# Arbol-Project/dcdf

Hardware: AMD Instinct MI355X
Metric: raster cells/s encoded (Snapshot+Log build) (higher is better)
Workload: dtype int32; 1 GPU; configs[2]: 4096x4096x365 i32 raster, seed 0xDCDF0003, tiled into 3072 [<=32,256,256] chunks; 3072 of them on this GPU; workload_key=config2/i32/n3072/w1, chunks_total=3072, chunks_on_rank0=3072, cells_total=6123683840, k=2, device=gfx950:sramecc+:xnack- AMD Radeon Graphics, 256 CUs, failed_tiles_rank0=0, encoded_bytes_rank0=4115239087, snapshots_rank0=3072, bytes_verified_vs_oracle=0, parallelism=chunks sharded over 1 GPU(s), no data-path collective

## Files before the change

### dcdf_amd/csrc/k2r_encode.h

```cpp
#pragma once
#include "k2r_exec.h"


#ifndef K2R_DIAG_SKIP
#define K2R_DIAG_SKIP 0
#endif

namespace k2r {

template <int LOG2S>
struct EncCfg {
    static_assert(LOG2S >= 3 && LOG2S <= 8, "kernel body written for sidelen 8..256 (the library dispatches 16..256)");
    static constexpr int H = LOG2S;
    static constexpr int S = 1 << LOG2S;
    static constexpr int NBLK = 1 << (2 * (LOG2S - 3));
    static constexpr int NT = NBLK;
    static constexpr int NW = NT < 64 ? 1 : NT / 64;
    static constexpr int NTOP = ((1 << (2 * (H - 2))) - 1) / 3;
    static constexpr int NTOPX = NTOP - (1 << (2 * (H - 3)));
    static constexpr int TBW = (NTOPX + 31) / 32 + 1;
    static constexpr int MAXV = ((1 << (2 * (H + 1))) - 1) / 3;
    static constexpr int MAXT = ((1 << (2 * H)) - 1) / 3;
    static constexpr int WV = (MAXV + 31) / 32;
    static constexpr int WT = (MAXT + 31) / 32;
    static constexpr int top_off(int h) { return ((1 << (2 * (H - 2))) - (1 << (2 * (H - h + 1)))) / 3; }
    static constexpr int kWaveHeader = 1;
    static constexpr int kWavePrefix = 2;
};

struct EncRegs {
    uint32_t d2[4];
    uint32_t flags;
    uint32_t u2;
    uint32_t sc[MAX_SCAN_FIELDS];
    uint64_t pf_lo;
    uint32_t pf_l2;
    uint32_t pa[5];
#ifdef K2R_REGCOPY
    uint32_t cw[32];
#endif
};

K2R_HD uint32_t unpackI(int h, uint64_t lo, uint64_t top) {
    switch (h) {
        case 1: return (uint32_t)(lo & 0xffffu);
        case 2: return (uint32_t)((lo >> 16) & 0x3fffu);
        case 3: return (uint32_t)((lo >> 30) & 0xfffu);
        case 4: return (uint32_t)(top & 0x3ffu);
        case 5: return (uint32_t)((top >> 10) & 0xffu);
        case 6: return (uint32_t)((top >> 18) & 0x3fu);
// ... 511 lines not shown
};

template <class C>
struct EncShared : EncPool<C> {
    using EncPool<C>::POOL_L1;
    using EncPool<C>::POOL_BMV1;
    using EncPool<C>::POOL_PREFV;
    using EncPool<C>::POOLW;
    int32_t tmin[C::NTOP], tmax[C::NTOP], smin[C::NTOP], smax[C::NTOP], diff[C::NTOP];
    uint32_t eq[C::NTOP];
    uint32_t pool[EncPool<C>::POOLW];
    uint32_t bmT[C::WT + 1], bmE[C::WT + 1];
    uint32_t bmV0[C::WV + 1];
    uint32_t bmM[2][C::WT + 1];
    uint32_t prefM[C::WT + 2];
    uint32_t wsum[C::NW][MAX_SCAN_FIELDS];
    uint32_t tot[MAX_SCAN_FIELDS];
    K2R_HD uint32_t* L2() { return pool; }
    K2R_HD uint16_t* L1() { return (uint16_t*)(pool + POOL_L1); }
    K2R_HD uint32_t* bmV1() { return pool + POOL_BMV1; }
    K2R_HD uint32_t* prefV() { return pool + POOL_PREFV; }
    static constexpr int PREFTOP = 48;
    uint32_t prefTopV[PREFTOP + 1];
    uint32_t pfx[3][C::NBLK];
    uint32_t lq[C::NBLK][2];
    uint32_t li[C::NBLK];
    uint32_t tbS[C::TBW], tbL[C::TBW];
    uint32_t tbP[C::TBW + 1];
    uint32_t ttR[C::H + 2];
    uint32_t nlistV, nlistM;
    uint32_t stI, stQ;
    uint32_t tkI, tkQ;
    InstPlan<C> pl;
    int32_t err;
    uint32_t work;
    uint32_t fault[6];
    uint64_t prof[NPROF], prof_last;
#ifdef K2R_PROFILE
    uint64_t pw[16][NPROF][2];
#endif
};

template <class EX>
K2R_HD bool guard_ok(EX& ex, bool ok, uint32_t code, uint32_t inst, uint32_t tid, uint32_t value, uint32_t limit) {
    ex.gfail |= ok ? 0u : (1u << (code & 31u));
    (void)inst; (void)tid; (void)value; (void)limit;
    return ok;
}
template <bool UNIFORM_SPAN = true, class EX>
// ... 532 lines not shown
            o.su = 0;
#pragma unroll
            for (int q = 0; q < 4; q++) {
                x[q] = (uint32_t)((d[4 * q] ^ d[4 * q + 1]) | (d[4 * q] ^ d[4 * q + 2]) | (d[4 * q] ^ d[4 * q + 3]));
                const uint32_t u1 = nz((uint32_t)(mn1[q] ^ mx1[q]));
                o.pq[q] = u1 & nz(x[q]);
                o.tb1 = (o.tb1 << 1) | o.pq[q];
                o.e4 = (o.e4 << 1) | (u1 ^ o.pq[q]);
                o.su += u1;
                const uint32_t sxq = (q & 1) ? (sx[q >> 1] >> 16) : (sx[q >> 1] & 0xffffu);
                const uint32_t snq = (q & 1) ? (sn[q >> 1] >> 16) : (sn[q >> 1] & 0xffffu);
                o.recw[q] = pk_lo16((uint32_t)(mx1[q] - (int32_t)sxq), (uint32_t)(mn1[q] - (int32_t)snq));
                o.qw[2 * q] = pk_lo16((uint32_t)d[4 * q], (uint32_t)d[4 * q + 1]);
                o.qw[2 * q + 1] = pk_lo16((uint32_t)d[4 * q + 2], (uint32_t)d[4 * q + 3]);
            }
            const uint32_t X = x[0] | x[1] | x[2] | x[3] | (uint32_t)((d[0] ^ d[4]) | (d[0] ^ d[8]) | (d[0] ^ d[12]));
            o.ne2 = nz(X);
            o.nu2 = nz((uint32_t)(o.mn2 ^ o.mx2));
            o.p2 = o.ne2 & o.nu2;
            o.nq = popc32(o.tb1);
            o.d0 = d[0];
            o.d2w = pk_lo16((uint32_t)(o.mx2 - (int32_t)o.smx2), (uint32_t)(o.mn2 - (int32_t)o.smn2));
        };
        auto lean_put = [&](const LeanSub& o, uint32_t owner, uint32_t lI1b, uint32_t lI2b) {
            uint32_t slotQ, slotI, endQ, endI;
            ex.stash_alloc(o.nq | (o.p2 << 16), &sh.stQ, &sh.stI, slotQ, slotI, endQ, endI);
            uint32_t ord = lI1b;
            const uint32_t p0 = owner | (lI2b << 10) | (lI1b << 12) | (o.tb1 << 16) | (o.e4 << 20);
            if (endQ <= (uint32_t)SH::CAPQ_REC && endI <= (uint32_t)SH::CAPI_REC) {
#pragma unroll
                for (int q = 0; q < 4; q++) {
                    uint32_t* d = sh.pool + ((uint32_t)SH::QBASE + mul24(slotQ, 3u));
                    if (o.pq[q]) {
                        d[0] = owner | (ord << 10);
                        d[1] = o.qw[2 * q];
                        d[2] = o.qw[2 * q + 1];
                    }
                    slotQ += o.pq[q];
                    ord += o.pq[q];
                }
                if (o.p2) {
                    uint32_t* d = sh.pool + mul24(slotI, 5u);
                    d[0] = p0;
                    d[1] = o.recw[0];
                    d[2] = o.recw[1];
                    d[3] = o.recw[2];
                    d[4] = o.recw[3];
                }
            } else {
// ... 20 lines not shown
                        d[2] = o.recw[1];
                        d[3] = o.recw[2];
                        d[4] = o.recw[3];
                    } else {
                        gstore_words5(ovI + 5u * (slotI - (uint32_t)SH::CAPI_REC), p0, o.recw[0], o.recw[1], o.recw[2], o.recw[3]);
                    }
                }
            }
        };
        auto lean_block_out = [&](uint32_t B, int32_t mn3, int32_t mx3, uint32_t smn3, uint32_t smx3, int32_t dref, uint32_t Zb, uint32_t& wide,
                                  int32_t& err, bool store) {
            if (VEC == 1 && (mn3 < -VALUE_LIMIT || mx3 >= VALUE_LIMIT) && err == 0) err = ERR_RANGE;
            const int32_t smn3t = s_base + (int32_t)smn3, smx3t = s_base + (int32_t)smx3;
            wide = (mn3 - smx3t < -32768 || mx3 - smn3t > 32767) ? 1u : 0u;
            if (store) {
                sh.tmin[B] = mn3;
                sh.tmax[B] = mx3;
                if (s_build) {
                    sh.smin[B] = smn3t;
                    sh.smax[B] = smx3t;
                }
                sh.diff[B] = dref - s_base;
                sh.eq[B] = Zb == 0 ? 1u : 0u;
                sh.lq[B][0] = 0;
                sh.lq[B][1] = 0;
                sh.li[B] = 0;
            }
        };
        if (lean && !EX::kSim) {
            if constexpr (!EX::kSim) ex.par([&](int tid, EncRegs& r) {
                constexpr uint32_t NTW = NT < 64 ? NT : 64, BPP = NTW / 4;
                const uint32_t ltid = opaque((uint32_t)tid), lane = ltid & 63u, j = lane & 3u;
                int32_t err = 0;
                auto request_t = [&](int p, int32_t (&tt)[16]) {
                    const uint32_t Bp = (ltid & ~63u) + BPP * (uint32_t)p + (lane >> 2);
                    uint32_t br, bc;
                    morton_decode(4u * Bp + j, br, bc);
                    load_sub16<false, VEC>(ta, inst, 4u * br, 4u * bc, 0, tt, err);
                    if (VEC >= 2) err = (int32_t)opaque((uint32_t)err);
                };
                auto request_w = [&](int p, uint32_t (&ww)[8]) {
                    const uint32_t Bp = (ltid & ~63u) + BPP * (uint32_t)p + (lane >> 2);
#ifdef K2R_REGCOPY
#pragma unroll
                    for (int i = 0; i < 8; i++) ww[i] = r.cw[8 * p + i];
                    (void)Bp;
#else
                    load_compact_raw<C>(cmp, (int)Bp, (int)j, ww);
#endif
// ... 21 lines not shown
                    if (K2R_LEAN_PREFETCH != 1) request_w(p, w);
#pragma unroll
                    for (int i = 0; i < 16; i++) t[i] = tn[i];
                    if (K2R_LEAN_PREFETCH == 1) {
#pragma unroll
                        for (int i = 0; i < 8; i++) w[i] = wn[i];
                    }
                    if (p < 3) {
                        request_t(p + 1, tn);
                        if (K2R_LEAN_PREFETCH == 1) request_w(p + 1, wn);
                    }
                    sched_fence();
#else
                    request_t(p, t);
                    request_w(p, w);
#endif
                    LeanSub o;
                    lean_analyse(t, w, o);
                    sched_fence();
                    const uint32_t cnt = o.nq | (o.p2 << 8) | (o.su << 16) | (o.nu2 << 24);
                    const uint32_t n0 = EX::template quad_bcast<0>(cnt), n1 = EX::template quad_bcast<1>(cnt), n2 = EX::template quad_bcast<2>(cnt),
                                   n3 = EX::template quad_bcast<3>(cnt);
                    const uint32_t pre = (j > 0 ? n0 : 0u) + (j > 1 ? n1 : 0u) + (j > 2 ? n2 : 0u), tot = n0 + n1 + n2 + n3;
                    lean_put(o, B, pre & 0xffu, (pre >> 8) & 0xffu);
                    const int32_t mn3 = EX::quad_min(o.mn2), mx3 = EX::quad_max(o.mx2);
                    const uint32_t smn3 = (uint32_t)EX::quad_min((int32_t)o.smn2), smx3 = (uint32_t)EX::quad_max((int32_t)o.smx2);
                    const int32_t dref = (int32_t)EX::template quad_bcast<0>((uint32_t)o.d0);
                    const uint32_t Zb = EX::quad_or(o.ne2 | nz((uint32_t)(o.d0 ^ dref)));
                    uint32_t wide;
                    lean_block_out(B, mn3, mx3, smn3, smx3, dref, Zb, wide, err, j == 0);
                    const uint32_t fw = EX::quad_or(((o.ne2 ^ 1u) << j) | (o.su << (4u + 3u * j)) | (o.nq << (16u + 3u * j))) | (wide << 28);
                    const uint32_t uw = EX::quad_or((o.nu2 ^ 1u) << j);
                    const uint32_t own_lane = lane - BPP * (uint32_t)p, src = (4u * own_lane) & 63u;
                    const uint32_t g0 = EX::lane_pull(src, o.d2w), g1 = EX::lane_pull(src + 1u, o.d2w), g2 = EX::lane_pull(src + 2u, o.d2w),
                                   g3 = EX::lane_pull(src + 3u, o.d2w);
                    const uint32_t gf = EX::lane_pull(src, fw), gu = EX::lane_pull(src, uw), gt = EX::lane_pull(src, tot);
                    if (lane / BPP == (uint32_t)p) {
                        r.d2[0] = g0;
                        r.d2[1] = g1;
                        r.d2[2] = g2;
                        r.d2[3] = g3;
                        r.flags = gf;
                        r.u2 = gu;
                        r.sc[0] = ((gt >> 16) & 0xffu) | ((gt >> 24) << 16);
                        r.sc[3] = (gt & 0xffu) | (((gt >> 8) & 0xffu) << 16);
                    }
                }
// ... 4 lines not shown
                if (err != 0) ex.lds_min(&sh.err, err);
            });
        } else if (lean) ex.par([&](int tid, EncRegs& r) {
            uint32_t r0, c0;
            blk_origin(tid, r0, c0);
            int32_t err = 0;
            uint32_t sI1 = 0, sI2 = 0, lI1 = 0, lI2 = 0, eqbits = 0, cntbits = 0, u2 = 0, Z = 0;
            int32_t mn3 = 0, mx3 = 0, dref = 0;
            uint32_t smn3 = 0, smx3 = 0;
#pragma unroll
            for (int j = 0; j < 4; j++) {
                int32_t t[16];
                uint32_t w[8];
                load_sub16<false, VEC>(ta, inst, r0, c0, j, t, err);
#ifdef K2R_REGCOPY
                for (int i = 0; i < 8; i++) w[i] = r.cw[8 * j + i];
#else
                load_compact_raw<C>(cmp, tid, j, w);
#endif
                LeanSub o;
                lean_analyse(t, w, o);
                if (j == 0) dref = o.d0;
                Z |= o.ne2 | nz((uint32_t)(o.d0 ^ dref));
                lean_put(o, (uint32_t)tid, lI1, lI2);
                sI1 += o.su;
                sI2 += o.nu2;
                cntbits |= (o.su << (4 + 3 * j)) | (o.nq << (16 + 3 * j));
                lI1 += o.nq;
                lI2 += o.p2;
                u2 |= (o.nu2 ^ 1u) << j;
                eqbits |= (o.ne2 ^ 1u) << j;
                r.d2[j] = o.d2w;
                mn3 = j == 0 ? o.mn2 : (o.mn2 < mn3 ? o.mn2 : mn3);
                mx3 = j == 0 ? o.mx2 : (o.mx2 > mx3 ? o.mx2 : mx3);
                smn3 = j == 0 ? o.smn2 : (o.smn2 < smn3 ? o.smn2 : smn3);
                smx3 = j == 0 ? o.smx2 : (o.smx2 > smx3 ? o.smx2 : smx3);
            }
            uint32_t wide;
            lean_block_out((uint32_t)tid, mn3, mx3, smn3, smx3, dref, Z, wide, err, true);
            r.sc[0] = sI1 | (sI2 << 16);
            r.flags = eqbits | cntbits | (wide << 28);
            r.u2 = u2;
            if (tid < C::TBW) {
                sh.tbS[tid] = 0;
                sh.tbL[tid] = 0;
            }
            r.sc[3] = lI1 | (lI2 << 16);
            if (err != 0) ex.lds_min(&sh.err, err);
        });
        else ex.par([&](int tid, EncRegs& r) {
            uint32_t r0, c0;
            blk_origin(tid, r0, c0);
            int32_t err = 0;
            const bool inv3 = inval(r0, c0);
            uint32_t sI1 = 0, sI2 = 0, lI1 = 0, lI2 = 0;
            if (have_s) {
                sh.lq[tid][0] = 0;
                sh.lq[tid][1] = 0;
                sh.li[tid] = 0;
            }
            int32_t df2_0 = 0, mn3 = 0, mx3 = 0, smn3 = 0, smx3 = 0;
            uint32_t eqbits = 0, eqall = 1, cntbits = 0, wide = 0, u2 = 0;
#pragma unroll
            for (int j = 0; j < 4; j++) {
                sched_fence();
                const uint32_t rj = r0 + 4 * (j >> 1), cj = c0 + 4 * (j & 1);
                const bool inv2 = inval(rj, cj);
                int32_t t16[16];
                load_sub16<PADDED, VEC>(ta, inst, r0, c0, j, t16, err);
                int32_t mn1[4], mx1[4];
                bool inv1[4], P1S[4];
#pragma unroll
                for (int qq = 0; qq < 4; qq++) {
                    mn1[qq] = min4(t16[4 * qq], t16[4 * qq + 1], t16[4 * qq + 2], t16[4 * qq + 3]);
                    mx1[qq] = max4(t16[4 * qq], t16[4 * qq + 1], t16[4 * qq + 2], t16[4 * qq + 3]);
                    inv1[qq] = inval(rj + 2 * (qq >> 1), cj + 2 * (qq & 1));
                    P1S[qq] = !inv1[qq] && mn1[qq] != mx1[qq];
                    sI1 += P1S[qq] ? 1u : 0u;
                    cntbits += (P1S[qq] ? 1u : 0u) << (4 + 3 * j);
// ... 113 lines not shown
        ex.stamp(0);

        const bool rec_ovf = stI > (uint32_t)SH::CAPI_REC || stQ > (uint32_t)SH::CAPQ_REC;
        const uint32_t rec_corr = lean ? (uint32_t)s_base & 0xffffu : 0u;
        auto rec16 = [&](uint32_t half) -> int32_t { return (int32_t)(int16_t)(uint16_t)(half - rec_corr); };
        auto lng = [](int32_t v) -> uint32_t { return ((uint32_t)v + 128u) > 255u ? 1u : 0u; };
        auto top_node = [&](int h, int j) {
            const int c = C::top_off(h - 1) + 4 * j, a = C::top_off(h) + j;
            sh.tmin[a] = min4(sh.tmin[c], sh.tmin[c + 1], sh.tmin[c + 2], sh.tmin[c + 3]);
            sh.tmax[a] = max4(sh.tmax[c], sh.tmax[c + 1], sh.tmax[c + 2], sh.tmax[c + 3]);
            if (have_s) {
                if (s_build) {
                    sh.smin[a] = min4(sh.smin[c], sh.smin[c + 1], sh.smin[c + 2], sh.smin[c + 3]);
                    sh.smax[a] = max4(sh.smax[c], sh.smax[c + 1], sh.smax[c + 2], sh.smax[c + 3]);
                }
                const int32_t d0 = sh.diff[c];
                sh.diff[a] = d0;
                sh.eq[a] = (sh.eq[c] & sh.eq[c + 1] & sh.eq[c + 2] & sh.eq[c + 3]) && d0 == sh.diff[c + 1] && d0 == sh.diff[c + 2] &&
                                   d0 == sh.diff[c + 3]
                               ? 1u
                               : 0u;
            }
        };
        auto prepass = [&](uint32_t first, uint32_t step) {
            for (uint32_t m = first; m < stQ; m += step) {
                uint32_t q[3];
                if (m < (uint32_t)SH::CAPQ_REC) {
#pragma unroll
                    for (int i = 0; i < 3; i++) q[i] = sh.pool[SH::QBASE + 3u * m + i];
                } else {
                    gload_words<3>(ovQ + 3u * (m - (uint32_t)SH::CAPQ_REC), q);
                }
                const uint32_t own = q[0] & 1023u, ord = (q[0] >> 10) & 15u;
                const uint32_t f = lng(rec16(q[1] & 0xffffu)) | (lng(rec16(q[1] >> 16)) << 1) | (lng(rec16(q[2] & 0xffffu)) << 2) |
                                   (lng(rec16(q[2] >> 16)) << 3);
                if (f) ex.lds_or(&sh.lq[own][ord >> 3], f << (4u * (ord & 7u)));
            }
            for (uint32_t k = first; k < stI; k += step) {
                uint32_t rec[5];
                if (k < (uint32_t)SH::CAPI_REC) {
#pragma unroll
                    for (int i = 0; i < 5; i++) rec[i] = sh.pool[5u * k + i];
                } else {
                    gload_words<5>(ovI + 5u * (k - (uint32_t)SH::CAPI_REC), rec);
                }
                const uint32_t own = rec[0] & 1023u, ord2 = (rec[0] >> 10) & 3u, tb1 = (rec[0] >> 16) & 15u;
                uint32_t f = 0;
// ... 215 lines not shown
                }
            };
            const uint32_t wt = opaque((uint32_t)tid);
            node(3, wt);
            if (tid == 0) {
                sh.stI = 0;
                sh.stQ = 0;
                sh.tkI = 0;
                sh.tkQ = 0;
            }
            if (wt < (uint32_t)C::NTOPX) {
                int h;
                uint32_t j;
                top_decode(wt, h, j);
                node(h, j);
            }
            r.sc[1] = sI3 | (lI3 << 16);
            r.sc[2] = sTop;
            r.sc[4] = lTop;
            r.sc[5] = lMax.c1 | (lMin.c1 << 16);
            r.sc[6] = wide;
            uint32_t cL0 = 0, cL1 = 0, mL1 = 0, cL2 = 0, mL2 = 0;
            if (have_s) {
                const uint32_t fl = sh.li[tid];
                cL0 = popc32(sh.lq[tid][0]) + popc32(sh.lq[tid][1]);
                cL1 = popc32(fl & 0x0f0f0f0fu);
                mL1 = popc32(fl & 0xf0f0f0f0u);
#pragma unroll
                for (int j = 0; j < 4; j++) {
                    const int32_t vx = rec16(r.d2[j] & 0xffffu), vn = rec16(r.d2[j] >> 16);
                    r.d2[j] = ((uint32_t)vx & 0xffffu) | ((uint32_t)vn << 16);
                    const bool P2L = ((r.u2 >> j) & 1u) == 0 && ((r.flags >> j) & 1u) == 0;
                    cL2 += lI3 ? lng(vx) : 0u;
                    mL2 += P2L ? lng(vn) : 0u;
                }
            }
            r.sc[7] = cL0;
            r.sc[8] = cL1 | (cL2 << 16);
            r.sc[9] = mL1 | (mL2 << 16);
        });
        ex.stamp(2);
        ex.template scan_begin<10>();
        ex.stamp(3);

        auto classes_pass = [&](const int which) {
#ifdef K2R_SIM_TRACE
            if (EX::kSim) __builtin_printf("classes_pass(%d) inst=%u\n", which, inst);
#endif
            ex.par_nosync([&](int tid, EncRegs& r) {
                uint32_t r0, c0;
                blk_origin(tid, r0, c0);
                int32_t lerr = 0;
                Cls vMax, vMin;
                auto cnode = [&](int h, uint32_t j) {
                    if (which == 0) {
                        vMax.add(zz32(snap_vmax(h, j)), (h == H) ? true : PS(h + 1, j >> 2));
                        vMin.add(zz32(snap_vmin(h, j)), PS(h, j));
                    } else {
                        vMax.add(zz32(log_vmax(h, j)), (h == H) ? true : PL(h + 1, j >> 2));
                        vMin.add(zz32(log_vmin(h, j)), PL(h, j));
                    }
                };
                cnode(3, (uint32_t)tid);
                if (tid < C::NTOPX) {
                    int h;
// ... 60 lines not shown
                            const bool P1 = !unif1 && !(d[0] == d[1] && d[0] == d[2] && d[0] == d[3]);
                            vMax.add(zz32(inv1 ? 0 : mx1 - smx1), true);
                            vMin.add(zz32(mn1 - smn1), P1);
#pragma unroll
                            for (int i = 0; i < 4; i++) vMax.add(zz32(d[i]), P1);
                        }
                    }
                }
                r.sc[10] = vMax.c1;
                r.sc[11] = vMax.c2;
                r.sc[12] = vMax.c3;
                r.sc[13] = vMin.c1;
                r.sc[14] = vMin.c2;
                r.sc[15] = vMin.c3;
            });
            ex.template reduce<6, 10>();
        };

        const bool cap254 = have_s && (blk_count - 1 == 254);
        auto plan = [&](const int stage) {
            ex.par([&](int tid, EncRegs&) {
                uint32_t T10[10];
                if (stage == 1) {
                    ex.template scan_finish<10>(T10);
                    for (uint32_t w = (uint32_t)tid; w <= (uint32_t)C::WT; w += NT) {
                        sh.bmT[w] = 0;
                        sh.bmE[w] = 0;
                        sh.bmM[0][w] = 0;
                    }
                    for (uint32_t w = (uint32_t)tid; w <= (uint32_t)C::WV; w += NT) sh.bmV0[w] = 0;
                }
                constexpr bool kTwoLanes = !EX::kSim && NT >= 2;
                if (tid >= (stage == 1 && kTwoLanes ? 2 : 1)) return;
                auto& pl = sh.pl;
                auto choose = [&](bool snap, const Totals<C>& W, uint32_t size, uint32_t narrow) {
                    pl.as_snapshot = snap ? 1u : 0u;
                    pl.isize = size;
                    pl.use_stash = (!snap && narrow && 5u * stI + 3u * stQ <= stash_cap && stI == W.Ni[2] && stQ == W.Ni[1]) ? 1u : 0u;
                    uint32_t rr = 0;
#pragma unroll
                    for (int h = 4; h <= H; h++) {
                        sh.ttR[h] = rr;
                        rr += W.Ni[h];
                    }
                    sh.ttR[H + 1] = rr;
                };
                if (stage == 1) {
                    const uint32_t t0 = T10[0], t1 = T10[1], t2 = T10[2], t3 = T10[3], t4 = T10[4], t5 = T10[5], t6 = T10[6], t7 = T10[7],
                                   t8 = T10[8], t9 = T10[9];
                    const uint32_t narrow = (have_s && t6 == 0) ? 1u : 0u;
                    const uint32_t lv2 = t5 & 0xffffu, lv1 = lv2 + (t8 >> 16), lv0 = lv1 + (t8 & 0xffffu);
                    const uint32_t lm2 = t5 >> 16, lm1 = lm2 + (t9 >> 16);
                    auto cand = [&](uint32_t c, Totals<C>& T, DacLayout& V, DacLayout& M, uint32_t& eo) {
                        T.from(c == 0 ? ((uint64_t)t0 | ((uint64_t)(t1 & 0xffffu) << 30)) : ((uint64_t)t3 | ((uint64_t)(t1 >> 16) << 30)),
                               c == 0 ? t2 : t4);
                        eo = 13 + bitmap_size(T.LT);
                        const uint32_t vbase = c == 0 ? eo : eo + bitmap_size(T.LT - T.M0);
                        const bool counts = c == 1 && narrow;
                        V = dac_layout(vbase, T.N0, counts ? lv0 + t7 : 0u, 0, 0);
                        M = dac_layout(V.end, T.M0, counts ? lm1 + (t9 & 0xffffu) : 0u, 0, 0);
                    };
                    uint32_t snap_lb, log_size, eq_off;
                    Totals<C> TW;
                    bool i_hold_log;
                    if (kTwoLanes) {
                        DacLayout V, M;
                        uint32_t eo;
                        cand((uint32_t)tid, TW, V, M, eo);
                        if (tid == 0 || have_s) {
                            pl.T[tid] = TW;
                            pl.V[tid] = V;
                            pl.M[tid] = M;
                        }
// ... 93 lines not shown
            }
            blk_hdr = off;
            off += 1;
            blk_count = 0;
            s_idx = inst;
            n_snap++;
            const int32_t rmin = ex.uni(sh.tmin[C::top_off(H)]), rmax = ex.uni(sh.tmax[C::top_off(H)]);
            s_cmp = (int64_t)rmax - (int64_t)rmin <= 65535 && inst + 1 < ta.instants;
            s_base = rmin;
            cmp = (head && inst == 0) ? ta.shared_cmp : scmp;
        } else {
            n_log++;
        }
        if ((uint64_t)off + isize > cap) {
            status = ST_OUT_CAPACITY;
            break;
        }
        uint8_t* const io = out + off;
        n_stash += use_stash ? 1u : 0u;
        ex.stamp(12);
        ex.par([&](int tid, EncRegs& r) {
            const uint32_t pI12 = as_snapshot ? r.sc[0] : r.sc[3];
            const uint32_t pI3 = as_snapshot ? (r.sc[1] & 0xffffu) : (r.sc[1] >> 16);
            const uint32_t pL0 = r.sc[7], pL12 = r.sc[8], pM12 = r.sc[9];
            r.pf_lo = (uint64_t)pI12 | ((uint64_t)pI3 << 30);
            r.pf_l2 = (pL12 >> 16) | (pM12 & 0xffff0000u);
            sh.pfx[0][tid] = pI12;
            sh.pfx[1][tid] = pL0;
            sh.pfx[2][tid] = (pL12 & 0xffffu) | (pM12 << 16);
            const uint32_t tp = EX::item(tid, C::kWavePrefix), th = EX::item(tid, C::kWaveHeader);
            if (tp == 0) {
                const uint32_t* const tbw = as_snapshot ? sh.tbS : sh.tbL;
                uint32_t wd[C::TBW], run = 0;
#pragma unroll
                for (int w = 0; w < C::TBW; w++) wd[w] = tbw[w];
#pragma unroll
                for (int w = 0; w < C::TBW; w++) {
                    sh.tbP[w] = run;
                    run += popc32(wd[w]);
                }
                sh.tbP[C::TBW] = run;
            }
            if (th == 0) {
                sh.nlistV = 0;
                sh.nlistM = 0;
                if (do_patch) gstore8(out + hdr_patch_off, (uint8_t)hdr_patch_val);
                gstore8(io, 2);
                gstore32u(io + 1, __builtin_bswap32(ta.rows));
                gstore32u(io + 5, __builtin_bswap32(ta.cols));
                gstore32u(io + 9, __builtin_bswap32((uint32_t)C::S));
                gstore8(io + DV.bm_off[0] - 1, (uint8_t)DV.nlev);
                gstore8(io + DM.bm_off[0] - 1, (uint8_t)DM.nlev);
// ... 209 lines not shown
                    uint32_t w[4];
#pragma unroll
                    for (int qq = 0; qq < 4; qq++) w[qq] = rec[1 + qq];
                    const uint32_t p1 = offV1 + 4 * kk;
                    emit4<0, EM_ONE>(ex, sinkV, p1, zz32(rec16(w[0] & 0xffffu)), zz32(rec16(w[1] & 0xffffu)),
                                     zz32(rec16(w[2] & 0xffffu)), zz32(rec16(w[3] & 0xffffu)), tid,
                                     lv1 + (pl & 0xffffu) + popc32(below & 0x0f0f0f0fu));
                    bm_or_run(ex, sh.bmT, guard_pos(ex, p1, 4, lt, kGuardTRun1), 4, tb1);
                    bm_or_run(ex, sh.bmE, guard_pos<false>(ex, offZ1 + 4 * kk - pre, elen, ne, kGuardE1), elen, erun);
                    uint32_t n1 = 0, lm = lm1 + (pl >> 16) + popc32(below & 0xf0f0f0f0u);
#pragma unroll
                    for (int qq = 0; qq < 4; qq++) {
                        if ((tb1 >> (3 - qq)) & 1u) {
                            const uint32_t zm = zz32(rec16(w[qq] >> 16));
                            emit_val<1, EM_ONE>(ex, sinkM, offI1 + pre + n1, zm, tid, lm);
                            lm += zm > 0xffu ? 1u : 0u;
                            n1++;
                        }
                    }
                }
                guard_flush(ex);
              });
            };
            if (K2R_DIAG_SKIP & 2) {
            } else if (rec_ovf) passI(EmTag<1>{});
            else passI(EmTag<0>{});
            ex.stamp(11);
            auto passQ = [&](auto ovf_tag) {
              constexpr bool OVF = decltype(ovf_tag)::value != 0;
              ex.par([&](int tid, EncRegs&) {
                const uint32_t offV0 = TT.offV[0], lv0 = sh.pl.lngV[0];
                for (uint32_t m = ex.take(&sh.tkQ, tid); m < nI1; m = ex.take(&sh.tkQ, tid)) {
                    uint32_t q[3];
                    if (!OVF || m < (uint32_t)SH::CAPQ_REC) {
#pragma unroll
                        for (int i = 0; i < 3; i++) q[i] = sh.pool[SH::QBASE + 3u * m + i];
                    } else {
                        gload_words<3>(ovQ + 3u * (m - (uint32_t)SH::CAPQ_REC), q);
                    }
                    const uint32_t hdr = q[0], a = q[1], b = q[2];
                    const uint32_t own = hdr & 1023u;
                    const uint32_t ord = (hdr >> 10) & 15u;
                    const uint32_t pos = (sh.pfx[0][own] & 0xffffu) + ord;
                    const uint32_t f0 = sh.lq[own][0], f1 = sh.lq[own][1], cut = (1u << (4u * (ord & 7u))) - 1u;
                    const uint32_t before = ord < 8u ? popc32(f0 & cut) : popc32(f0) + popc32(f1 & cut);
                    emit4<0, EM_ONE>(ex, sinkV, offV0 + 4 * pos, zz32(rec16(a & 0xffffu)), zz32(rec16(a >> 16)),
                                     zz32(rec16(b & 0xffffu)), zz32(rec16(b >> 16)), tid, lv0 + sh.pfx[1][own] + before);
                }
                guard_flush(ex);
              });
            };
            if (K2R_DIAG_SKIP & 4) ex.barrier();
            else if (rec_ovf) passQ(EmTag<1>{});
            else passQ(EmTag<0>{});
            ex.stamp(6);
            {
                const uint32_t lt = ex.uni(TT.LT), m0 = ex.uni(TT.M0);
                const BmJob jobs[4] = {{sh.bmT, lt, nullptr, 0, io + 13},
                                       {sh.bmE, lt - m0, nullptr, 0, io + log_eq_off},
                                       {sh.bmV0, sinkV.n0, sh.prefTopV, SH::PREFTOP, nlevV > 0 ? io + ex.uni(DV.bm_off[0]) : nullptr},
                                       {sh.bmM[0], sinkM.n0, sh.prefM, SH::PREFTOP, nlevM > 0 ? io + ex.uni(DM.bm_off[0]) : nullptr}};
                if (!(K2R_DIAG_SKIP & 8)) bitmaps_finish<C, 4>(ex, jobs);
            }
            ex.stamp(8);
            if (nlevV > 1 || nlevM > 1) {
                if (!(K2R_DIAG_SKIP & 16)) ex.par_nosync([&](int tid, EncRegs& r) {
                    auto put = [&](const DacSink& d, uint32_t* bm0, uint32_t pos, uint32_t hi) {
                        if (hi) {
                            pos = guard_pos(ex, pos, 1, d.n0 < 32u * SH::PREFTOP ? d.n0 : 32u * SH::PREFTOP, d.code);
                            gstore8(d.plane1 + guard_pos(ex, bm_rank(bm0, d.pref, pos), 1, d.n1, d.code + 1), (uint8_t)hi);
                        }
                    };
                    const uint32_t hb = r.pa[2];
                    put(sinkV, sh.bmV0, r.pa[0], hb & 0xffu);
                    put(sinkM, sh.bmM[0], r.pa[1], (hb >> 8) & 0xffu);
// ... 185 lines not shown
```

### dcdf_amd/csrc/k2r_exec.h

```cpp
#pragma once
#include "k2r_common.h"

namespace k2r {

constexpr int MAX_SCAN_FIELDS = 16;

template <int NT>
K2R_HD constexpr uint32_t wave_item(int tid, int rot) {
    constexpr uint32_t NW = NT <= 64 ? 1u : (uint32_t)NT / 64u;
    return NT <= 64 ? (uint32_t)tid : ((((uint32_t)tid >> 6) + (uint32_t)rot) % NW) * 64u + ((uint32_t)tid & 63u);
}
template <int NT>
K2R_HD constexpr int wave_rot_to(int v) {
    constexpr int NW = NT <= 64 ? 1 : NT / 64;
    return (NW - v % NW) % NW;
}

#if defined(__HIPCC__)

template <class SH, class TR, int NT>
struct GpuExec {
    SH& sh;
    TR r;
    const int tid;
    uint32_t gfail = 0;
    static constexpr int kNT = NT;
    static constexpr bool kSim = false;

    __device__ GpuExec(SH& s) : sh(s), tid((int)threadIdx.x) {}
    __device__ __forceinline__ static uint32_t item(int t, int first) { return wave_item<NT>(t, wave_rot_to<NT>(first)); }

#ifdef K2R_PROFILE
    uint64_t pw_last = 0, pw_work = 0, pw_wait = 0;
    __device__ __forceinline__ void pw_before() {
        const uint64_t t = __builtin_amdgcn_s_memtime();
        pw_work += t - pw_last;
        pw_last = t;
    }
    __device__ __forceinline__ void pw_after() {
        const uint64_t t = __builtin_amdgcn_s_memtime();
        pw_wait += t - pw_last;
        pw_last = t;
    }
    __device__ __forceinline__ void pw_start() { pw_last = __builtin_amdgcn_s_memtime(); pw_work = pw_wait = 0; }
#else
    __device__ __forceinline__ void pw_before() {}
    __device__ __forceinline__ void pw_after() {}
    __device__ __forceinline__ void pw_start() {}
#endif

// ... 222 lines not shown
        x |= row_ror<4>(x);
        return x | row_ror<8>(x);
    }
    __device__ __forceinline__ static int32_t wave_min_of_rows(int32_t x) {
        const int32_t a = __builtin_amdgcn_readlane(x, 0), b = __builtin_amdgcn_readlane(x, 16), c = __builtin_amdgcn_readlane(x, 32),
                      d = __builtin_amdgcn_readlane(x, 48);
        const int32_t p = a < b ? a : b, q = c < d ? c : d;
        return p < q ? p : q;
    }
    __device__ __forceinline__ static int32_t wave_max_of_rows(int32_t x) {
        const int32_t a = __builtin_amdgcn_readlane(x, 0), b = __builtin_amdgcn_readlane(x, 16), c = __builtin_amdgcn_readlane(x, 32),
                      d = __builtin_amdgcn_readlane(x, 48);
        const int32_t p = a > b ? a : b, q = c > d ? c : d;
        return p > q ? p : q;
    }
    __device__ __forceinline__ static uint32_t wave_or_of_rows(uint32_t x) {
        return (uint32_t)(__builtin_amdgcn_readlane((int)x, 0) | __builtin_amdgcn_readlane((int)x, 16) | __builtin_amdgcn_readlane((int)x, 32) |
                          __builtin_amdgcn_readlane((int)x, 48));
    }
    __device__ __forceinline__ static uint32_t lane_pull(uint32_t src, uint32_t v) {
        return (uint32_t)__builtin_amdgcn_ds_bpermute((int)(src << 2), (int)v);
    }

    __device__ __forceinline__ void stash_alloc(uint32_t c, uint32_t* cntA, uint32_t* cntB, uint32_t& a, uint32_t& b, uint32_t& enda,
                                                uint32_t& endb) {
        constexpr int W = NT < 64 ? NT : 64;
        const int lane = tid & 63;
        const uint32_t incl = wave_incl_scan(c);
        const uint32_t tot = (uint32_t)__builtin_amdgcn_readlane((int)incl, W - 1);
        uint32_t ret = 0;
        if (lane < 2) ret = atomicAdd(lane == 0 ? cntA : cntB, lane == 0 ? (tot & 0xffffu) : (tot >> 16));
        const uint32_t ba = (uint32_t)__builtin_amdgcn_readlane((int)ret, 0), bb = (uint32_t)__builtin_amdgcn_readlane((int)ret, W > 1 ? 1 : 0);
        const uint32_t excl = incl - c;
        a = ba + (excl & 0xffffu);
        b = bb + (excl >> 16);
        enda = ba + (tot & 0xffffu);
        endb = bb + (tot >> 16);
    }

    __device__ __forceinline__ uint32_t take(uint32_t* ctr, int t) {
        constexpr uint32_t W = NT < 64 ? NT : 64;
        uint32_t first = 0;
        if ((t & 63) == 0) first = atomicAdd(ctr, W);
        return (uint32_t)__builtin_amdgcn_readfirstlane((int)first) + (uint32_t)(t & 63);
    }

    __device__ __forceinline__ uint32_t lds_or_nr(uint32_t* p, uint32_t v) { atomicOr(p, v); return 0; }
    __device__ __forceinline__ uint32_t lds_or(uint32_t* p, uint32_t v) { return atomicOr(p, v); }
    __device__ __forceinline__ uint32_t lds_add(uint32_t* p, uint32_t v) { return atomicAdd(p, v); }
    __device__ __forceinline__ int32_t lds_min(int32_t* p, int32_t v) { return atomicMin(p, v); }

    template <int NF, bool TOT = true>
    __device__ __forceinline__ void scan() {
        constexpr int W = NT < 64 ? NT : 64;
        constexpr int NW = NT < 64 ? 1 : NT / 64;
        const int lane = tid & 63;
        const int wave = __builtin_amdgcn_readfirstlane(tid >> 6);
        int incl[NF];
#pragma unroll
        for (int f = 0; f < NF; f++) incl[f] = (int)r.sc[f];
        wave_incl_scan_n(incl);
        if (lane == W - 1) {
#pragma unroll
            for (int f = 0; f < NF; f++) sh.wsum[wave][f] = (uint32_t)incl[f];
        }
        lds_barrier();
        int x[NF];
// ... 5 lines not shown
            const uint32_t tot = (uint32_t)__builtin_amdgcn_readlane(x[f], NW - 1);
            const uint32_t base = wave == 0 ? 0u : (uint32_t)__builtin_amdgcn_readlane(x[f], wave - 1);
            r.sc[f] = base + (uint32_t)incl[f] - r.sc[f];
            if (TOT && tid == 0) sh.tot[f] = tot;
        }
        if (TOT) lds_barrier();
    }
};

#endif

#if !defined(__HIP_DEVICE_COMPILE__)
}
#include <vector>
namespace k2r {

template <class SH, class TR, int NT>
struct SimExec {
    SH& sh;
    std::vector<TR> regs;
    uint32_t gfail = 0;
    static constexpr int kNT = NT;
    static constexpr bool kSim = true;

    explicit SimExec(SH& s) : sh(s), regs(NT) {}
    static uint32_t item(int t, int first) { return wave_item<NT>(t, wave_rot_to<NT>(first)); }

    template <class F>
    void par(F&& f) {
        for (int t = 0; t < NT; t++) f(t, regs[t]);
    }
    template <class F>
    void par_nosync(F&& f) {
        for (int t = 0; t < NT; t++) f(t, regs[t]);
    }
    void barrier() {}
    template <int P>
    void prio() {}
    void wave_lds_fence() {}
    void barrier_global() {}
    void publish(uint32_t* flag, uint32_t value, uint32_t payload) {
        flag[1] = payload;
        flag[0] = value;
    }
    uint32_t await(const uint32_t* flag, uint32_t timeout_value) { return flag[0] != 0 ? flag[0] : timeout_value; }
    uint32_t flag_payload(const uint32_t* flag) { return flag[1]; }
// ... 1 lines not shown
    template <class T>
    T uni(T v) const { return v; }
    template <int NF, int F0 = 0>
    void reduce() {
        for (int f = F0; f < F0 + NF; f++) {
            uint32_t run = 0;
            for (int t = 0; t < NT; t++) run += regs[t].sc[f];
            sh.tot[f] = run;
        }
    }

    template <int NF>
    void scan_begin() {
        scan<NF, true>();
    }
    static constexpr int planner() { return 0; }
    uint32_t lane_value(uint32_t v, int) const { return v; }
    template <int NF>
    void scan_finish(uint32_t (&t)[NF]) {
        for (int f = 0; f < NF; f++) t[f] = sh.tot[f];
    }


    void stash_alloc(uint32_t c, uint32_t* cntA, uint32_t* cntB, uint32_t& a, uint32_t& b, uint32_t& enda, uint32_t& endb) {
        a = *cntA;
        b = *cntB;
        *cntA += c & 0xffffu;
        *cntB += c >> 16;
        enda = *cntA;
        endb = *cntB;
    }
    uint32_t take(uint32_t* ctr, int) { return (*ctr)++; }
    uint32_t lds_or_nr(uint32_t* p, uint32_t v) {
        *p |= v;
        return 0;
    }
    uint32_t lds_or(uint32_t* p, uint32_t v) {
        uint32_t o = *p;
        *p = o | v;
        return o;
    }
    uint32_t lds_add(uint32_t* p, uint32_t v) {
        uint32_t o = *p;
        *p = o + v;
        return o;
    }
    int32_t lds_min(int32_t* p, int32_t v) {
        int32_t o = *p;
        if (v < o) *p = v;
        return o;
    }

    template <int NF, bool TOT = true>
    void scan() {
        for (int f = 0; f < NF; f++) {
// ... 14 lines not shown
```

Measured before the change: 596.6 billion cells/s.

## Compute level-1/level-0 stash prefixes by wave tickets instead of per-block LDS tables

For the non-padded path, the per-block lq/li bitmask tables and the two extra scan fields are replaced by per-wave run tables recorded at stash allocation. A prepass scans stash records in wave-sized tickets, then a line scan turns the ticket totals into level offsets, and new passI/passQ level variants emit directly in stash order using these ticket prefixes. The aim is to cut LDS traffic, scan width and scattered per-block bookkeeping. In exchange it adds a prepass over all records, walk_slot lookups and a union that reuses LDS storage, which raises the risk of aliasing errors.

```diff
diff --git a/dcdf_amd/csrc/k2r_encode.h b/dcdf_amd/csrc/k2r_encode.h
--- a/dcdf_amd/csrc/k2r_encode.h
+++ b/dcdf_amd/csrc/k2r_encode.h
@@ -26,6 +26,7 @@
     static constexpr int top_off(int h) { return ((1 << (2 * (H - 2))) - (1 << (2 * (H - h + 1)))) / 3; }
     static constexpr int kWaveHeader = 1;
     static constexpr int kWavePrefix = 2;
+    static constexpr int kWaveTickets = 3;
 };
 
 struct EncRegs {
@@ -583,9 +584,21 @@
     K2R_HD uint32_t* prefV() { return pool + POOL_PREFV; }
     static constexpr int PREFTOP = 48;
     uint32_t prefTopV[PREFTOP + 1];
-    uint32_t pfx[3][C::NBLK];
-    uint32_t lq[C::NBLK][2];
-    uint32_t li[C::NBLK];
+    static constexpr int WL = C::NT < kWaveLanes ? C::NT : kWaveLanes;
+    static constexpr int NRUN = 4 * C::NT / WL;
+    static constexpr int TKQ = 16 * C::NBLK / WL + 1, TKI = 4 * C::NBLK / WL + 1;
+    union {
+        struct {
+            uint32_t pfx[3][C::NBLK];
+            uint32_t lq[C::NBLK][2];
+            uint32_t li[C::NBLK];
+        };
+        struct {
+            uint32_t runQ[NRUN], runI[NRUN];
+            uint32_t tq[TKQ], ti[2][TKI];
+            uint32_t lvlTot[3];
+        };
+    };
     uint32_t tbS[C::TBW], tbL[C::TBW];
     uint32_t tbP[C::TBW + 1];
     uint32_t ttR[C::H + 2];
@@ -1164,9 +1177,9 @@
             o.d0 = d[0];
             o.d2w = pk_lo16((uint32_t)(o.mx2 - (int32_t)o.smx2), (uint32_t)(o.mn2 - (int32_t)o.smn2));
         };
-        auto lean_put = [&](const LeanSub& o, uint32_t owner, uint32_t lI1b, uint32_t lI2b) {
+        auto lean_put = [&](const LeanSub& o, uint32_t owner, uint32_t lI1b, uint32_t lI2b, uint32_t run) {
             uint32_t slotQ, slotI, endQ, endI;
-            ex.stash_alloc(o.nq | (o.p2 << 16), &sh.stQ, &sh.stI, slotQ, slotI, endQ, endI);
+            ex.stash_alloc(o.nq | (o.p2 << 16), &sh.stQ, &sh.stI, &sh.runQ[run], &sh.runI[run], slotQ, slotI, endQ, endI);
             uint32_t ord = lI1b;
             const uint32_t p0 = owner | (lI2b << 10) | (lI1b << 12) | (o.tb1 << 16) | (o.e4 << 20);
             if (endQ <= (uint32_t)SH::CAPQ_REC && endI <= (uint32_t)SH::CAPI_REC) {
@@ -1233,9 +1246,6 @@
                 }
                 sh.diff[B] = dref - s_base;
                 sh.eq[B] = Zb == 0 ? 1u : 0u;
-                sh.lq[B][0] = 0;
-                sh.lq[B][1] = 0;
-                sh.li[B] = 0;
             }
         };
         if (lean && !EX::kSim) {
@@ -1303,7 +1313,7 @@
                     const uint32_t n0 = EX::template quad_bcast<0>(cnt), n1 = EX::template quad_bcast<1>(cnt), n2 = EX::template quad_bcast<2>(cnt),
                                    n3 = EX::template quad_bcast<3>(cnt);
                     const uint32_t pre = (j > 0 ? n0 : 0u) + (j > 1 ? n1 : 0u) + (j > 2 ? n2 : 0u), tot = n0 + n1 + n2 + n3;
-                    lean_put(o, B, pre & 0xffu, (pre >> 8) & 0xffu);
+                    lean_put(o, B, pre & 0xffu, (pre >> 8) & 0xffu, 4u * (ltid >> 6) + (uint32_t)p);
                     const int32_t mn3 = EX::quad_min(o.mn2), mx3 = EX::quad_max(o.mx2);
                     const uint32_t smn3 = (uint32_t)EX::quad_min((int32_t)o.smn2), smx3 = (uint32_t)EX::quad_max((int32_t)o.smx2);
                     const int32_t dref = (int32_t)EX::template quad_bcast<0>((uint32_t)o.d0);
@@ -1354,7 +1364,7 @@
                 lean_analyse(t, w, o);
                 if (j == 0) dref = o.d0;
                 Z |= o.ne2 | nz((uint32_t)(o.d0 ^ dref));
-                lean_put(o, (uint32_t)tid, lI1, lI2);
+                lean_put(o, (uint32_t)tid, lI1, lI2, 4u * (uint32_t)tid + (uint32_t)j);
                 sI1 += o.su;
                 sI2 += o.nu2;
                 cntbits |= (o.su << (4 + 3 * j)) | (o.nq << (16 + 3 * j));
@@ -1386,7 +1396,7 @@
             int32_t err = 0;
             const bool inv3 = inval(r0, c0);
             uint32_t sI1 = 0, sI2 = 0, lI1 = 0, lI2 = 0;
-            if (have_s) {
+            if (PADDED && have_s) {
                 sh.lq[tid][0] = 0;
                 sh.lq[tid][1] = 0;
                 sh.li[tid] = 0;
@@ -1546,7 +1556,71 @@
                                : 0u;
             }
         };
+        auto load_q = [&](uint32_t slot, uint32_t n, uint32_t (&q)[3]) {
+            slot = slot < n ? slot : 0u;
+            if (!rec_ovf || slot < (uint32_t)SH::CAPQ_REC) {
+#pragma unroll
+                for (int i = 0; i < 3; i++) q[i] = sh.pool[SH::QBASE + 3u * slot + i];
+            } else {
+                gload_words<3>(ovQ + 3u * (slot - (uint32_t)SH::CAPQ_REC), q);
+            }
+        };
+        auto load_i = [&](uint32_t slot, uint32_t n, uint32_t (&rec)[5]) {
+            slot = slot < n ? slot : 0u;
+            if (!rec_ovf || slot < (uint32_t)SH::CAPI_REC) {
+#pragma unroll
+                for (int i = 0; i < 5; i++) rec[i] = sh.pool[5u * slot + i];
+            } else {
+                gload_words<5>(ovI + 5u * (slot - (uint32_t)SH::CAPI_REC), rec);
+            }
+        };
+        auto i_counts = [&](const uint32_t (&rec)[5], uint32_t& cx, uint32_t& cn, uint32_t& nq) {
+            const uint32_t tb1 = (rec[0] >> 16) & 15u;
+            cx = cn = 0;
+#pragma unroll
+            for (int qq = 0; qq < 4; qq++) {
+                cx += lng(rec16(rec[1 + qq] & 0xffffu));
+                cn += ((tb1 >> (3 - qq)) & 1u) & lng(rec16(rec[1 + qq] >> 16));
+            }
+            nq = popc32(tb1);
+        };
+        auto prepass_level = [&](uint32_t first, uint32_t step) {
+            constexpr uint32_t W = (uint32_t)EX::kW;
+            const uint32_t lane = first % W, nwv = step / W, wv = ex.uni(nwv - 1u - first / W);
+            const uint32_t nTQ = (stQ + W - 1u) / W, nTI = (stI + W - 1u) / W;
+            auto wq = ex.walk_load(sh.runQ, SH::NRUN);
+            auto wi = ex.walk_load(sh.runI, SH::NRUN);
+            for (uint32_t c = wv; c < nTQ + nTI; c += nwv) {
+                if (c < nTQ) {
+                    const uint32_t L0 = c * W, L = L0 + lane;
+                    uint32_t q[3];
+                    load_q(ex.walk_slot(wq, L0, L), stQ, q);
+                    int f[1] = {L < stQ ? (int)(lng(rec16(q[1] & 0xffffu)) + lng(rec16(q[1] >> 16)) + lng(rec16(q[2] & 0xffffu)) +
+                                                lng(rec16(q[2] >> 16)))
+                                        : 0};
+                    uint32_t tot[1];
+                    EX::wave_excl_scan_n(f, tot);
+                    if (lane == 0) sh.tq[c] = tot[0];
+                } else {
+                    const uint32_t t = c - nTQ, L0 = t * W, L = L0 + lane;
+                    uint32_t rec[5], cx, cn, nq;
+                    load_i(ex.walk_slot(wi, L0, L), stI, rec);
+                    i_counts(rec, cx, cn, nq);
+                    int f[2] = {L < stI ? (int)(cx | (cn << 16)) : 0, L < stI ? (int)nq : 0};
+                    uint32_t tot[2];
+                    EX::wave_excl_scan_n(f, tot);
+                    if (lane == 0) {
+                        sh.ti[0][t] = tot[0];
+                        sh.ti[1][t] = tot[1];
+                    }
+                }
+            }
+        };
         auto prepass = [&](uint32_t first, uint32_t step) {
+            if constexpr (!PADDED) {
+                if (lean) prepass_level(first, step);
+                return;
+            }
             for (uint32_t m = first; m < stQ; m += step) {
                 uint32_t q[3];
                 if (m < (uint32_t)SH::CAPQ_REC) {
@@ -1808,10 +1882,12 @@
             r.sc[6] = wide;
             uint32_t cL0 = 0, cL1 = 0, mL1 = 0, cL2 = 0, mL2 = 0;
             if (have_s) {
-                const uint32_t fl = sh.li[tid];
-                cL0 = popc32(sh.lq[tid][0]) + popc32(sh.lq[tid][1]);
-                cL1 = popc32(fl & 0x0f0f0f0fu);
-                mL1 = popc32(fl & 0xf0f0f0f0u);
+                if constexpr (PADDED) {
+                    const uint32_t fl = sh.li[tid];
+                    cL0 = popc32(sh.lq[tid][0]) + popc32(sh.lq[tid][1]);
+                    cL1 = popc32(fl & 0x0f0f0f0fu);
+                    mL1 = popc32(fl & 0xf0f0f0f0u);
+                }
 #pragma unroll
                 for (int j = 0; j < 4; j++) {
                     const int32_t vx = rec16(r.d2[j] & 0xffffu), vn = rec16(r.d2[j] >> 16);
@@ -1821,12 +1897,24 @@
                     mL2 += P2L ? lng(vn) : 0u;
                 }
             }
-            r.sc[7] = cL0;
-            r.sc[8] = cL1 | (cL2 << 16);
-            r.sc[9] = mL1 | (mL2 << 16);
+            if constexpr (PADDED) {
+                r.sc[7] = cL0;
+                r.sc[8] = cL1 | (cL2 << 16);
+                r.sc[9] = mL1 | (mL2 << 16);
+            } else {
+                r.sc[7] = cL2 | (mL2 << 16);
+                if (lean && EX::item(tid, C::kWaveTickets) < (uint32_t)EX::kW) {
+                    constexpr uint32_t W = (uint32_t)EX::kW;
+                    const uint32_t nTQ = (stQ + W - 1u) / W, nTI = (stI + W - 1u) / W;
+                    ex.line_excl_scan(sh.tq, nTQ, &sh.lvlTot[0]);
+                    ex.line_excl_scan(sh.ti[0], nTI, &sh.lvlTot[1]);
+                    ex.line_excl_scan(sh.ti[1], nTI, &sh.lvlTot[2]);
+                }
+            }
         });
         ex.stamp(2);
-        ex.template scan_begin<10>();
+        constexpr int NSCAN = PADDED ? 10 : 8;
+        ex.template scan_begin<NSCAN>();
         ex.stamp(3);
 
         auto classes_pass = [&](const int which) {
@@ -1933,7 +2021,18 @@
             ex.par([&](int tid, EncRegs&) {
                 uint32_t T10[10];
                 if (stage == 1) {
-                    ex.template scan_finish<10>(T10);
+                    if constexpr (PADDED) {
+                        ex.template scan_finish<10>(T10);
+                    } else {
+                        uint32_t T8[8];
+                        ex.template scan_finish<8>(T8);
+#pragma unroll
+                        for (int f = 0; f < 7; f++) T10[f] = T8[f];
+                        const uint32_t l1 = lean ? sh.lvlTot[1] : 0u;
+                        T10[7] = lean ? sh.lvlTot[0] : 0u;
+                        T10[8] = (l1 & 0xffffu) | (T8[7] << 16);
+                        T10[9] = (l1 >> 16) | (T8[7] & 0xffff0000u);
+                    }
                     for (uint32_t w = (uint32_t)tid; w <= (uint32_t)C::WT; w += NT) {
                         sh.bmT[w] = 0;
                         sh.bmE[w] = 0;
@@ -1959,7 +2058,7 @@
                 if (stage == 1) {
                     const uint32_t t0 = T10[0], t1 = T10[1], t2 = T10[2], t3 = T10[3], t4 = T10[4], t5 = T10[5], t6 = T10[6], t7 = T10[7],
                                    t8 = T10[8], t9 = T10[9];
-                    const uint32_t narrow = (have_s && t6 == 0) ? 1u : 0u;
+                    const uint32_t narrow = (have_s && t6 == 0 && (PADDED || lean)) ? 1u : 0u;
                     const uint32_t lv2 = t5 & 0xffffu, lv1 = lv2 + (t8 >> 16), lv0 = lv1 + (t8 & 0xffffu);
                     const uint32_t lm2 = t5 >> 16, lm1 = lm2 + (t9 >> 16);
                     auto cand = [&](uint32_t c, Totals<C>& T, DacLayout& V, DacLayout& M, uint32_t& eo) {
@@ -2099,12 +2198,16 @@
         ex.par([&](int tid, EncRegs& r) {
             const uint32_t pI12 = as_snapshot ? r.sc[0] : r.sc[3];
             const uint32_t pI3 = as_snapshot ? (r.sc[1] & 0xffffu) : (r.sc[1] >> 16);
-            const uint32_t pL0 = r.sc[7], pL12 = r.sc[8], pM12 = r.sc[9];
             r.pf_lo = (uint64_t)pI12 | ((uint64_t)pI3 << 30);
-            r.pf_l2 = (pL12 >> 16) | (pM12 & 0xffff0000u);
-            sh.pfx[0][tid] = pI12;
-            sh.pfx[1][tid] = pL0;
-            sh.pfx[2][tid] = (pL12 & 0xffffu) | (pM12 << 16);
+            if constexpr (PADDED) {
+                const uint32_t pL0 = r.sc[7], pL12 = r.sc[8], pM12 = r.sc[9];
+                r.pf_l2 = (pL12 >> 16) | (pM12 & 0xffff0000u);
+                sh.pfx[0][tid] = pI12;
+                sh.pfx[1][tid] = pL0;
+                sh.pfx[2][tid] = (pL12 & 0xffffu) | (pM12 << 16);
+            } else {
+                r.pf_l2 = r.sc[7];
+            }
             const uint32_t tp = EX::item(tid, C::kWavePrefix), th = EX::item(tid, C::kWaveHeader);
             if (tp == 0) {
                 const uint32_t* const tbw = as_snapshot ? sh.tbS : sh.tbL;
@@ -2360,8 +2463,55 @@
                 guard_flush(ex);
               });
             };
+            auto passI_level = [&]() {
+              ex.par_nosync([&](int tid, EncRegs&) {
+                constexpr uint32_t W = (uint32_t)EX::kW;
+                const uint32_t offV1 = TT.offV[1], offZ1 = TT.offZ[1], offI1 = TT.offI[1], lt = TT.LT, ne = TT.LT - TT.M0;
+                const uint32_t lv1 = sh.pl.lngV[1], lm1 = sh.pl.lngM[1], lane = (uint32_t)tid % W;
+                auto wi = ex.walk_load(sh.runI, SH::NRUN);
+                for (uint32_t k0 = ex.take_first(&sh.tkI, tid); k0 < nI2; k0 = ex.take_first(&sh.tkI, tid)) {
+                    const uint32_t kk = k0 + lane, t = k0 / W;
+                    const bool live = kk < nI2;
+                    uint32_t rec[5], cx, cn, nq;
+                    load_i(ex.walk_slot(wi, k0, kk), nI2, rec);
+                    i_counts(rec, cx, cn, nq);
+                    int f[2] = {live ? (int)(cx | (cn << 16)) : 0, live ? (int)nq : 0};
+                    uint32_t tot[2];
+                    EX::wave_excl_scan_n(f, tot);
+                    const uint32_t pl = sh.ti[0][t] + (uint32_t)f[0];
+                    const uint32_t pre = sh.ti[1][t] + (uint32_t)f[1];
+                    if (live) {
+                        const uint32_t hdr = rec[0];
+                        const uint32_t tb1 = (hdr >> 16) & 15u, e4 = (hdr >> 20) & 15u, elen = 4u - nq;
+                        uint32_t erun = 0;
+#pragma unroll
+                        for (int qq = 0; qq < 4; qq++) {
+                            const uint32_t t0 = ((tb1 >> (3 - qq)) & 1u) ^ 1u;
+                            erun = (erun << t0) | ((e4 >> (3 - qq)) & t0);
+                        }
+                        const uint32_t p1 = offV1 + 4 * kk;
+                        emit4<0, EM_ONE>(ex, sinkV, p1, zz32(rec16(rec[1] & 0xffffu)), zz32(rec16(rec[2] & 0xffffu)),
+                                         zz32(rec16(rec[3] & 0xffffu)), zz32(rec16(rec[4] & 0xffffu)), tid, lv1 + (pl & 0xffffu));
+                        bm_or_run(ex, sh.bmT, guard_pos(ex, p1, 4, lt, kGuardTRun1), 4, tb1);
+                        bm_or_run(ex, sh.bmE, guard_pos<false>(ex, offZ1 + 4 * kk - pre, elen, ne, kGuardE1), elen, erun);
+                        uint32_t n1 = 0, lm = lm1 + (pl >> 16);
+#pragma unroll
+                        for (int qq = 0; qq < 4; qq++) {
+                            if ((tb1 >> (3 - qq)) & 1u) {
+                                const uint32_t zm = zz32(rec16(rec[1 + qq] >> 16));
+                                emit_val<1, EM_ONE>(ex, sinkM, offI1 + pre + n1, zm, tid, lm);
+                                lm += zm > 0xffu ? 1u : 0u;
+                                n1++;
+                            }
+                        }
+                    }
+                }
+                guard_flush(ex);
+              });
+            };
             if (K2R_DIAG_SKIP & 2) {
-            } else if (rec_ovf) passI(EmTag<1>{});
+            } else if constexpr (!PADDED) passI_level();
+            else if (rec_ovf) passI(EmTag<1>{});
             else passI(EmTag<0>{});
             ex.stamp(11);
             auto passQ = [&](auto ovf_tag) {
@@ -2388,7 +2538,28 @@
                 guard_flush(ex);
               });
             };
+            auto passQ_level = [&]() {
+              ex.par([&](int tid, EncRegs&) {
+                constexpr uint32_t W = (uint32_t)EX::kW;
+                const uint32_t offV0 = TT.offV[0], lv0 = sh.pl.lngV[0], lane = (uint32_t)tid % W;
+                auto wq = ex.walk_load(sh.runQ, SH::NRUN);
+                for (uint32_t m0 = ex.take_first(&sh.tkQ, tid); m0 < nI1; m0 = ex.take_first(&sh.tkQ, tid)) {
+                    const uint32_t m = m0 + lane;
+                    const bool live = m < nI1;
+                    uint32_t q[3];
+                    load_q(ex.walk_slot(wq, m0, m), nI1, q);
+                    const uint32_t z0 = zz32(rec16(q[1] & 0xffffu)), z1 = zz32(rec16(q[1] >> 16)), z2 = zz32(rec16(q[2] & 0xffffu)),
+                                   z3 = zz32(rec16(q[2] >> 16));
+                    int f[1] = {live ? (int)((z0 > 0xffu ? 1u : 0u) + (z1 > 0xffu ? 1u : 0u) + (z2 > 0xffu ? 1u : 0u) + (z3 > 0xffu ? 1u : 0u)) : 0};
+                    uint32_t tot[1];
+                    EX::wave_excl_scan_n(f, tot);
+                    if (live) emit4<0, EM_ONE>(ex, sinkV, offV0 + 4 * m, z0, z1, z2, z3, tid, lv0 + sh.tq[m0 / W] + (uint32_t)f[0]);
+                }
+                guard_flush(ex);
+              });
+            };
             if (K2R_DIAG_SKIP & 4) ex.barrier();
+            else if constexpr (!PADDED) passQ_level();
             else if (rec_ovf) passQ(EmTag<1>{});
             else passQ(EmTag<0>{});
             ex.stamp(6);
diff --git a/dcdf_amd/csrc/k2r_exec.h b/dcdf_amd/csrc/k2r_exec.h
--- a/dcdf_amd/csrc/k2r_exec.h
+++ b/dcdf_amd/csrc/k2r_exec.h
@@ -4,6 +4,12 @@
 namespace k2r {
 
 constexpr int MAX_SCAN_FIELDS = 16;
+
+#if defined(__HIPCC__)
+constexpr int kWaveLanes = 64;
+#else
+constexpr int kWaveLanes = 1;
+#endif
 
 template <int NT>
 K2R_HD constexpr uint32_t wave_item(int tid, int rot) {
@@ -26,6 +32,7 @@
     uint32_t gfail = 0;
     static constexpr int kNT = NT;
     static constexpr bool kSim = false;
+    static constexpr int kW = NT < 64 ? NT : 64;
 
     __device__ GpuExec(SH& s) : sh(s), tid((int)threadIdx.x) {}
     __device__ __forceinline__ static uint32_t item(int t, int first) { return wave_item<NT>(t, wave_rot_to<NT>(first)); }
@@ -294,14 +301,18 @@
         return (uint32_t)__builtin_amdgcn_ds_bpermute((int)(src << 2), (int)v);
     }
 
-    __device__ __forceinline__ void stash_alloc(uint32_t c, uint32_t* cntA, uint32_t* cntB, uint32_t& a, uint32_t& b, uint32_t& enda,
-                                                uint32_t& endb) {
+    __device__ __forceinline__ void stash_alloc(uint32_t c, uint32_t* cntA, uint32_t* cntB, uint32_t* runA, uint32_t* runB, uint32_t& a,
+                                                uint32_t& b, uint32_t& enda, uint32_t& endb) {
         constexpr int W = NT < 64 ? NT : 64;
         const int lane = tid & 63;
         const uint32_t incl = wave_incl_scan(c);
         const uint32_t tot = (uint32_t)__builtin_amdgcn_readlane((int)incl, W - 1);
         uint32_t ret = 0;
-        if (lane < 2) ret = atomicAdd(lane == 0 ? cntA : cntB, lane == 0 ? (tot & 0xffffu) : (tot >> 16));
+        if (lane < 2) {
+            const uint32_t mine = lane == 0 ? (tot & 0xffffu) : (tot >> 16);
+            ret = atomicAdd(lane == 0 ? cntA : cntB, mine);
+            *(lane == 0 ? runA : runB) = ret | (mine << 16);
+        }
         const uint32_t ba = (uint32_t)__builtin_amdgcn_readlane((int)ret, 0), bb = (uint32_t)__builtin_amdgcn_readlane((int)ret, W > 1 ? 1 : 0);
         const uint32_t excl = incl - c;
         a = ba + (excl & 0xffffu);
@@ -315,6 +326,58 @@
         uint32_t first = 0;
         if ((t & 63) == 0) first = atomicAdd(ctr, W);
         return (uint32_t)__builtin_amdgcn_readfirstlane((int)first) + (uint32_t)(t & 63);
+    }
+
+    __device__ __forceinline__ uint32_t take_first(uint32_t* ctr, int t) {
+        uint32_t first = 0;
+        if ((t & 63) == 0) first = atomicAdd(ctr, (uint32_t)kW);
+        return (uint32_t)__builtin_amdgcn_readfirstlane((int)first);
+    }
+
+    struct Walk {
+        uint32_t end, delta;
+    };
+    __device__ __forceinline__ Walk walk_load(const uint32_t* run, int nrun) {
+        static_assert(NT >= 4, "a wave holds its workgroup's run table: four runs per wave");
+        const int lane = tid & 63;
+        const uint32_t w = lane < nrun ? run[lane < nrun ? lane : 0] : 0u;
+        const uint32_t end = wave_incl_scan(w >> 16);
+        return Walk{end, (w & 0xffffu) - (end - (w >> 16))};
+    }
+    __device__ __forceinline__ uint32_t walk_slot(const Walk& wk, uint32_t L0, uint32_t L) const {
+        uint32_t g = (uint32_t)__builtin_amdgcn_readfirstlane((int)popc64(__builtin_amdgcn_ballot_w64(wk.end <= L0)));
+        uint32_t slot = 0, b = L0;
+        for (;;) {
+            const uint32_t e = (uint32_t)__builtin_amdgcn_readlane((int)wk.end, (int)g), d = (uint32_t)__builtin_amdgcn_readlane((int)wk.delta, (int)g);
+            slot = (L >= b && L < e) ? L + d : slot;
+            b = e;
+            if (e >= L0 + (uint32_t)kW || ++g >= (uint32_t)kW) break;
+        }
+        return slot;
+    }
+    template <int N>
+    __device__ __forceinline__ static void wave_excl_scan_n(int (&x)[N], uint32_t (&tot)[N]) {
+        int inc[N];
+#pragma unroll
+        for (int i = 0; i < N; i++) inc[i] = x[i];
+        wave_incl_scan_n(inc);
+#pragma unroll
+        for (int i = 0; i < N; i++) {
+            tot[i] = (uint32_t)__builtin_amdgcn_readlane(inc[i], kW - 1);
+            x[i] = inc[i] - x[i];
+        }
+    }
+    __device__ __forceinline__ void line_excl_scan(uint32_t* a, uint32_t n, uint32_t* total) {
+        const uint32_t lane = (uint32_t)tid & 63u;
+        uint32_t carry = 0;
+        for (uint32_t i0 = 0; i0 < n; i0 += (uint32_t)kW) {
+            const uint32_t i = i0 + lane;
+            const uint32_t v = i < n ? a[i] : 0u;
+            const uint32_t inc = wave_incl_scan(v);
+            if (i < n) a[i] = carry + inc - v;
+            carry += (uint32_t)__builtin_amdgcn_readlane((int)inc, kW - 1);
+        }
+        if (lane == 0) *total = carry;
     }
 
     __device__ __forceinline__ uint32_t lds_or_nr(uint32_t* p, uint32_t v) { atomicOr(p, v); return 0; }
@@ -366,6 +429,7 @@
     uint32_t gfail = 0;
     static constexpr int kNT = NT;
     static constexpr bool kSim = true;
+    static constexpr int kW = 1;
 
     explicit SimExec(SH& s) : sh(s), regs(NT) {}
     static uint32_t item(int t, int first) { return wave_item<NT>(t, wave_rot_to<NT>(first)); }
@@ -413,15 +477,45 @@
     }
 
 
-    void stash_alloc(uint32_t c, uint32_t* cntA, uint32_t* cntB, uint32_t& a, uint32_t& b, uint32_t& enda, uint32_t& endb) {
+    void stash_alloc(uint32_t c, uint32_t* cntA, uint32_t* cntB, uint32_t* runA, uint32_t* runB, uint32_t& a, uint32_t& b, uint32_t& enda,
+                     uint32_t& endb) {
         a = *cntA;
         b = *cntB;
         *cntA += c & 0xffffu;
         *cntB += c >> 16;
         enda = *cntA;
         endb = *cntB;
+        *runA = a | ((c & 0xffffu) << 16);
+        *runB = b | ((c >> 16) << 16);
     }
     uint32_t take(uint32_t* ctr, int) { return (*ctr)++; }
+    uint32_t take_first(uint32_t* ctr, int) { return (*ctr)++; }
+    struct Walk {
+        const uint32_t* run;
+        uint32_t nrun, g, base;
+    };
+    Walk walk_load(const uint32_t* run, int nrun) { return Walk{run, (uint32_t)nrun, 0u, 0u}; }
+    uint32_t walk_slot(Walk& wk, uint32_t, uint32_t L) const {
+        if (L < wk.base) wk.g = wk.base = 0;
+        while (wk.g < wk.nrun && L >= wk.base + (wk.run[wk.g] >> 16)) wk.base += wk.run[wk.g++] >> 16;
+        return wk.g < wk.nrun ? (wk.run[wk.g] & 0xffffu) + (L - wk.base) : 0u;
+    }
+    template <int N>
+    static void wave_excl_scan_n(int (&x)[N], uint32_t (&tot)[N]) {
+        for (int i = 0; i < N; i++) {
+            tot[i] = (uint32_t)x[i];
+            x[i] = 0;
+        }
+    }
+    void line_excl_scan(uint32_t* a, uint32_t n, uint32_t* total) {
+        uint32_t run = 0;
+        for (uint32_t i = 0; i < n; i++) {
+            const uint32_t v = a[i];
+            a[i] = run;
+            run += v;
+        }
+        *total = run;
+    }
     uint32_t lds_or_nr(uint32_t* p, uint32_t v) {
         *p |= v;
         return 0;
```

Result: slower. 530.9 billion cells/s (-11.0%).
